# ShigemichiMatsuzaki/MSPL

Measured on AMD Instinct MI355X. Metric: images/sec pseudo-label gen, ESPDNet-UE s=2.0 480x360(->288x480) bs=16, higher is better.
Workload: dtype f32; 1 GPU; BASELINE configs[1]: ESPDNet-UE s=2.0 C=13 single-source pseudo-label gen (forward + pred+0.5aux argmax + KL uncertainty + histogram), bs=16/GPU, 16x3x288x480 fp32, hipGraph replay, 3 launches in flight per GPU, 2 consecutive batches of 16 per launch; per_gpu_batch=16, batches_in_flight=3, batches_per_launch=2, classes=13

## Files before the change

mspl_amd/csrc/pyrpool_stream.hip:

```cpp
#include <stdlib.h>

#include <algorithm>

#include "common.hpp"
#include "pyr_stencil.hpp"

namespace mspl {

constexpr int P3_MAXB = 5;
#ifndef P3_STEPS
#define P3_STEPS 2
#endif
constexpr int P3_SEGMAX = 19;

struct Pyr3Geom {
    int N, P, h, w;
    int hs[P3_MAXB], ws[P3_MAXB];
    float sh[P3_MAXB], sw[P3_MAXB];
    int SEG, nseg, ncb, CBW;
    unsigned total;
};

template <int T, int PXL>
__device__ __forceinline__ void p3_up_branch(const float (&xw)[5][PXL + 4], const float* __restrict__ Arow,
                                             const float (&C)[3][PXL][5], float (&b)[PXL]) {
    constexpr int R0 = (5 - T) / 2;
    constexpr int NCOL = PXL + T - 1;
#pragma unroll
    for (int ky = 0; ky < 3; ++ky) {
        float a[5];
        {
            const float4 t4 = *reinterpret_cast<const float4*>(Arow + ky * 8);
            a[0] = t4.x; a[1] = t4.y; a[2] = t4.z; a[3] = t4.w;
            a[4] = T > 4 ? Arow[ky * 8 + 4] : 0.f;
        }
        float cs[NCOL];
#pragma unroll
        for (int s = 0; s < NCOL; ++s) {
            float v = a[0] * xw[R0][R0 + s];
#pragma unroll
            for (int rr = 1; rr < T; ++rr) v = fmaf(a[rr], xw[R0 + rr][R0 + s], v);
            cs[s] = v;
        }
#pragma unroll
        for (int j = 0; j < PXL; ++j) {
            float v = b[j];
#pragma unroll
            for (int s = 0; s < T; ++s) v = fmaf(C[ky][j][s], cs[j + s], v);
            b[j] = v;
        }
    }
}

template <int PXL> struct P3Vec;
template <> struct P3Vec<1> { typedef float T; };
template <> struct P3Vec<2> { typedef float2 T; };

template <int T0, int T1, int PXL, bool TRAIN>
__global__ __launch_bounds__(256, 2) void pyrpool_stream_kernel(const float* __restrict__ x, const float* __restrict__ sw0,
                                                                const float* __restrict__ sw1, const float* __restrict__ sw2,
                                                                const float* __restrict__ de3, const float* __restrict__ de4,
                                                                const float* __restrict__ br_scale, const float* __restrict__ br_shift,
                                                                const float* __restrict__ br_alpha, const float* __restrict__ merge_w,
                                                                const float* __restrict__ ep_scale,
                                                                const float* __restrict__ ep_shift,
                                                                const float* __restrict__ ep_alpha, int ep_ctot, int ep_coff,
                                                                Pyr3Geom g, float* __restrict__ out, float* __restrict__ zcat,
                                                                float* __restrict__ mraw) {
    __shared__ __attribute__((aligned(16))) float At[2][(P3_SEGMAX + 2) * 24];
    __shared__ float Gt[2][3][PXL][5][64];
    __shared__ __attribute__((aligned(16))) float Wm[4][5][12];
    const int lane = threadIdx.x & 63, wave = __builtin_amdgcn_readfirstlane(threadIdx.x >> 6);
    unsigned bid = blockIdx.x;
    const int sgi = bid % g.nseg;  bid /= g.nseg;
    const int cb = bid % g.ncb;  bid /= g.ncb;
    const int plane = (int)bid * 4 + wave;
    const int n = plane / g.P, c = plane - n * g.P;
    const int h = g.h, w = g.w;
    const int ys = sgi * g.SEG, ye = min(ys + g.SEG, h);
    const int px0 = cb * g.CBW + (lane - 1) * PXL;
    const bool writer = lane >= 1 && lane <= 62 && px0 < w;

    if (wave < 2) {
        const int ri = lane / 3, ky = lane - 3 * ri;
        if (ri < g.SEG + 2) {
            float acc[5];
            if (wave == 0) p3_coeffs<T0>(ys - 1 + ri, ky, h, g.hs[0], g.sh[0], acc);
            else p3_coeffs<T1>(ys - 1 + ri, ky, h, g.hs[1], g.sh[1], acc);
            float* d = &At[wave][ri * 24 + ky * 8];
            d[0] = acc[0]; d[1] = acc[1]; d[2] = acc[2]; d[3] = acc[3]; d[4] = acc[4];
        }
    }
#pragma unroll
    for (int t = 0; t < 6 * PXL; ++t) {
        if ((t & 3) == wave) {
            const int ub = t / (3 * PXL), r = t - ub * 3 * PXL, kx = r / PXL, j = r - kx * PXL;
            float acc[5];
            if (ub == 0) p3_coeffs<T0>(px0 + j, kx, w, g.ws[0], g.sw[0], acc);
            else p3_coeffs<T1>(px0 + j, kx, w, g.ws[1], g.sw[1], acc);
#pragma unroll
            for (int q = 0; q < 5; ++q) Gt[ub][kx][j][q][lane] = acc[q];
        }
    }
    __syncthreads();
    float C0[3][PXL][5], C1[3][PXL][5];
    {
        const float* w0p = sw0 + (size_t)c * 9;
        const float* w1p = sw1 + (size_t)c * 9;
#pragma unroll
        for (int j = 0; j < PXL; ++j)
#pragma unroll
            for (int s2 = 0; s2 < 5; ++s2) {
                const float a0 = Gt[0][0][j][s2][lane], a1 = Gt[0][1][j][s2][lane], a2 = Gt[0][2][j][s2][lane];
                const float b0 = Gt[1][0][j][s2][lane], b1 = Gt[1][1][j][s2][lane], b2 = Gt[1][2][j][s2][lane];
#pragma unroll
                for (int ky = 0; ky < 3; ++ky) {
                    C0[ky][j][s2] = fmaf(w0p[ky * 3 + 2], a2, fmaf(w0p[ky * 3 + 1], a1, w0p[ky * 3] * a0));
                    C1[ky][j][s2] = fmaf(w1p[ky * 3 + 2], b2, fmaf(w1p[ky * 3 + 1], b1, w1p[ky * 3] * b0));
                }
            }
    }
    unsigned dxa[2][PXL], dxb[2][PXL];  float dw0[2][PXL], dw1[2][PXL];
#pragma unroll
    for (int i = 0; i < 2; ++i)
#pragma unroll
        for (int j = 0; j < PXL; ++j) {
            const int px = min(max(px0 + j, 0), w - 1);
            int xa, xb;
            bilinear_src(g.sw[3 + i], px, g.ws[3 + i], xa, xb, dw0[i][j], dw1[i][j]);
            dxa[i][j] = (unsigned)xa * 4u;  dxb[i][j] = (unsigned)xb * 4u;
        }
    const float* wsame = sw2 + (size_t)c * 9;
    if (lane < 45) Wm[wave][lane / 9][lane % 9] = merge_w[(size_t)c * 45 + lane];
    const float4* wmq = reinterpret_cast<const float4*>(&Wm[wave][0][0]);
    float bsc[5], bsh[5], bal[5];
#pragma unroll
    for (int i = 0; i < 5; ++i) { bsc[i] = br_scale[i * g.P + c]; bsh[i] = br_shift[i * g.P + c]; bal[i] = br_alpha[i * g.P + c]; }
    const int cabs = ep_coff + c;
    const float esc = ep_scale ? ep_scale[cabs] : 1.f, esh = ep_shift ? ep_shift[cabs] : 0.f, eal = ep_alpha ? ep_alpha[cabs] : 1.f;
    const unsigned plane_id = __builtin_amdgcn_readfirstlane((unsigned)(n * g.P + c));
    const float* xpl = x + (size_t)plane_id * (size_t)(h * w);
    const float* e3 = de3 + (size_t)plane_id * (size_t)(g.hs[3] * g.ws[3]);
    const float* e4 = de4 + (size_t)plane_id * (size_t)(g.hs[4] * g.ws[4]);
    float* opl = out + ((size_t)__builtin_amdgcn_readfirstlane((unsigned)(n * ep_ctot + cabs))) * (size_t)(h * w);
    bool colin[PXL];
#pragma unroll
    for (int j = 0; j < PXL; ++j) colin[j] = px0 + j >= 0 && px0 + j < w;

    constexpr unsigned P3_OOB = 0x7ffffff0u;
    unsigned xoff[PXL + 4];
#pragma unroll
    for (int j = 0; j < PXL + 4; ++j) {
        const int cx = px0 - 2 + j;
        xoff[j] = (cx >= 0 && cx < w) ? (unsigned)cx * 4u : P3_OOB;
    }
    auto load_row = [&](int r, float (&v)[PXL + 4]) {
        const bool rin = r >= 0 && r < h;
        const float* row = xpl + (size_t)(rin ? r : 0) * w;
        const __amdgpu_buffer_rsrc_t rs = __builtin_amdgcn_make_buffer_rsrc(const_cast<float*>(row), 0, rin ? w * 4 : 0, 0x00020000);
        if (PXL == 2) {
#pragma unroll
            for (int j = 0; j < PXL + 4; j += 2) {
                typedef unsigned u32x2 __attribute__((ext_vector_type(2)));
                const u32x2 t = __builtin_amdgcn_raw_buffer_load_b64(rs, xoff[j], 0, 0);
                v[j] = __uint_as_float(t.x);  v[j + 1] = __uint_as_float(t.y);
            }
        } else {
#pragma unroll
            for (int j = 0; j < PXL + 4; ++j) v[j] = __uint_as_float(__builtin_amdgcn_raw_buffer_load_b32(rs, xoff[j], 0, 0));
        }
    };

    float xw[5][PXL + 4];
#pragma unroll
    for (int rr = 0; rr < 5; ++rr) load_row(ys - 3 + rr, xw[rr]);
    float en[2][PXL][4];
    float enwy0[2], enwy1[2];
    auto load_e = [&](int r) {
#pragma unroll
        for (int i = 0; i < 2; ++i) {
            int ya, yb;
            bilinear_src(g.sh[3 + i], min(max(r, 0), h - 1), g.hs[3 + i], ya, yb, enwy0[i], enwy1[i]);
            const int rowb = g.ws[3 + i] * 4;
            const __amdgpu_buffer_rsrc_t ra = __builtin_amdgcn_make_buffer_rsrc(const_cast<float*>((i == 0 ? e3 : e4) + ya * g.ws[3 + i]), 0, rowb, 0x00020000);
            const __amdgpu_buffer_rsrc_t rb = __builtin_amdgcn_make_buffer_rsrc(const_cast<float*>((i == 0 ? e3 : e4) + yb * g.ws[3 + i]), 0, rowb, 0x00020000);
#pragma unroll
            for (int j = 0; j < PXL; ++j) {
                en[i][j][0] = __uint_as_float(__builtin_amdgcn_raw_buffer_load_b32(ra, dxa[i][j], 0, 0));
                en[i][j][1] = __uint_as_float(__builtin_amdgcn_raw_buffer_load_b32(ra, dxb[i][j], 0, 0));
                en[i][j][2] = __uint_as_float(__builtin_amdgcn_raw_buffer_load_b32(rb, dxa[i][j], 0, 0));
                en[i][j][3] = __uint_as_float(__builtin_amdgcn_raw_buffer_load_b32(rb, dxb[i][j], 0, 0));
            }
        }
    };
    load_e(ys - 1);
    float acc[3][PXL];
#pragma unroll
    for (int r = 0; r < 3; ++r)
#pragma unroll
        for (int j = 0; j < PXL; ++j) acc[r][j] = 0.f;

    auto row_step = [&](const int br) __attribute__((always_inline)) {
        float bv[5][PXL];
        const bool rowin = br >= 0 && br < h;
        float ecur[2][PXL][4], wy0c[2], wy1c[2];
#pragma unroll
        for (int i = 0; i < 2; ++i) {
            wy0c[i] = enwy0[i]; wy1c[i] = enwy1[i];
#pragma unroll
            for (int j = 0; j < PXL; ++j)
#pragma unroll
                for (int q = 0; q < 4; ++q) ecur[i][j][q] = en[i][j][q];
        }
        if (br < ye) load_e(br + 1);
        float xn[PXL + 4];
        load_row(br + 3, xn);
        __builtin_amdgcn_sched_barrier(0);
        if (rowin) {
            const float* A0 = &At[0][(br - (ys - 1)) * 24];
            const float* A1 = &At[1][(br - (ys - 1)) * 24];
#pragma unroll
            for (int j = 0; j < PXL; ++j) { bv[0][j] = 0.f; bv[1][j] = 0.f; bv[2][j] = 0.f; }
            p3_up_branch<T0, PXL>(xw, A0, C0, bv[0]);
            p3_up_branch<T1, PXL>(xw, A1, C1, bv[1]);
#pragma unroll
            for (int ky = 0; ky < 3; ++ky) {
                const float w0 = wsame[ky * 3], w1 = wsame[ky * 3 + 1], w2 = wsame[ky * 3 + 2];
#pragma unroll
                for (int j = 0; j < PXL; ++j) {
                    bv[2][j] = fmaf(w0, xw[1 + ky][j + 1], bv[2][j]);
                    bv[2][j] = fmaf(w1, xw[1 + ky][j + 2], bv[2][j]);
                    bv[2][j] = fmaf(w2, xw[1 + ky][j + 3], bv[2][j]);
                }
            }
#pragma unroll
            for (int i = 0; i < 2; ++i)
#pragma unroll
                for (int j = 0; j < PXL; ++j) {
                    const float top = dw0[i][j] * ecur[i][j][0] + dw1[i][j] * ecur[i][j][1];
                    const float bot = dw0[i][j] * ecur[i][j][2] + dw1[i][j] * ecur[i][j][3];
                    bv[3 + i][j] = wy0c[i] * top + wy1c[i] * bot;
                }
            if (TRAIN && writer && br >= ys && br < ye) {
#pragma unroll
                for (int i = 0; i < 5; ++i) {
                    float* zp = zcat + (((size_t)n * 5 + i) * g.P + c) * (size_t)h * w + (size_t)br * w + px0;
                    if (PXL == 2) *reinterpret_cast<float2*>(zp) = make_float2(bv[i][0], bv[i][PXL - 1]);
                    else zp[0] = bv[i][0];
                }
            }
#pragma unroll
            for (int i = 0; i < 5; ++i)
#pragma unroll
                for (int j = 0; j < PXL; ++j) {
                    float v = fmaf(bv[i][j], bsc[i], bsh[i]);
                    v = v > 0.f ? v : bal[i] * v;
                    bv[i][j] = colin[j] ? v : 0.f;
                }
        } else {
#pragma unroll
            for (int i = 0; i < 5; ++i)
#pragma unroll
                for (int j = 0; j < PXL; ++j) bv[i][j] = 0.f;
        }
#pragma unroll
        for (int i = 0; i < 5; ++i) {
            float bx[PXL + 2];
            bx[0] = p3_from_left(bv[i][PXL - 1]);
#pragma unroll
            for (int j = 0; j < PXL; ++j) bx[1 + j] = bv[i][j];
            bx[PXL + 1] = p3_from_right(bv[i][0]);
            const float4 q0 = wmq[i * 3], q1 = wmq[i * 3 + 1], q2 = wmq[i * 3 + 2];
            const float wv[12] = {q0.x, q0.y, q0.z, q0.w, q1.x, q1.y, q1.z, q1.w, q2.x, q2.y, q2.z, q2.w};
#pragma unroll
            for (int r = 0; r < 3; ++r) {
                const int ky = 2 - r;
                const float w0 = wv[ky * 3], w1 = wv[ky * 3 + 1], w2 = wv[ky * 3 + 2];
#pragma unroll
                for (int j = 0; j < PXL; ++j) {
                    acc[r][j] = fmaf(w0, bx[j], acc[r][j]);
                    acc[r][j] = fmaf(w1, bx[j + 1], acc[r][j]);
                    acc[r][j] = fmaf(w2, bx[j + 2], acc[r][j]);
                }
            }
        }
#pragma unroll
        for (int rr = 0; rr < 4; ++rr)
#pragma unroll
            for (int j = 0; j < PXL + 4; ++j) xw[rr][j] = xw[rr + 1][j];
#pragma unroll
        for (int j = 0; j < PXL + 4; ++j) xw[4][j] = xn[j];
        const int y = br - 1;
        if (y >= ys) {
            float v[PXL];
#pragma unroll
            for (int j = 0; j < PXL; ++j) {
                v[j] = fmaf(acc[0][j], esc, esh);
                v[j] = (ep_alpha && v[j] <= 0.f) ? eal * v[j] : v[j];
            }
            if (writer) {
                float* dst = opl + (size_t)y * w + px0;
                if (PXL == 2) store_out2(dst, make_float2(v[0], v[PXL - 1]));
                else dst[0] = v[0];
                if (TRAIN) {
                    float* rp = mraw + ((size_t)n * g.P + c) * (size_t)h * w + (size_t)y * w + px0;
                    if (PXL == 2) *reinterpret_cast<float2*>(rp) = make_float2(acc[0][0], acc[0][PXL - 1]);
                    else rp[0] = acc[0][0];
                }
            }
        }
#pragma unroll
        for (int j = 0; j < PXL; ++j) { acc[0][j] = acc[1][j]; acc[1][j] = acc[2][j]; acc[2][j] = 0.f; }
    };
    constexpr int STEPS = TRAIN ? 2 : P3_STEPS;
#pragma unroll 1
    for (int br = ys - 1; br <= ye; br += STEPS) {
        row_step(br);
#pragma unroll
        for (int u = 1; u < STEPS; ++u)
            if (br + u <= ye) row_step(br + u);
    }
}

int pyrpool_stream_try(const float* x, int N, int P, int h, int w, int nb, const int32_t* hs, const int32_t* ws,
                       const float* const* stage_w, const float* const* down_e, const float* br_scale,
                       const float* br_shift, const float* br_alpha, const float* merge_w, const Epi& e, float* out,
                       hipStream_t stream, float* zcat) {
    static const int off = (MSPL_TUNE_INT("MSPL_PYR_STREAM", 1) == 0);
    static const int min_w = MSPL_TUNE_INT("MSPL_PYR_STREAM_MINW", 40);
    if (off || nb != 5 || w < min_w || ((int64_t)N * P) % 4 != 0) return 1;
    if (e.pre_add || e.residual || e.reinf_r || e.gate) return 1;
    for (int i = 0; i < 5; ++i) if (hs[i] <= 0 || ws[i] <= 0) return 1;
    if (!(hs[0] > h && ws[0] > w && hs[1] > h && ws[1] > w)) return 1;
    if (!(hs[2] == h && ws[2] == w)) return 1;
    if (!(hs[3] <= h && ws[3] <= w && hs[4] <= h && ws[4] <= w && (hs[3] < h || ws[3] < w) && (hs[4] < h || ws[4] < w))) return 1;
    if (!stage_w[0] || !stage_w[1] || !stage_w[2] || !down_e[3] || !down_e[4]) return 1;
    int taps[2];
    for (int i = 0; i < 2; ++i) {
        const int R = std::max(p3_stencil_radius(h, hs[i]), p3_stencil_radius(w, ws[i]));
        if (R > 2) return 1;
        taps[i] = R <= 1 ? 3 : 5;
    }
    const int PXL = w <= 62 ? 1 : 2;
    if (PXL == 2 && ((w & 1) || (((uintptr_t)out) & 7) || (((uintptr_t)x) & 7))) return 1;
    if (zcat && (!e.raw || e.ctot != P || e.coff != 0)) return 1;
    if (zcat && PXL == 2 && ((((uintptr_t)zcat) | ((uintptr_t)e.raw)) & 7)) return 1;
    Pyr3Geom g;
    memset(&g, 0, sizeof(g));
    g.N = N; g.P = P; g.h = h; g.w = w;
    for (int i = 0; i < 5; ++i) {
        g.hs[i] = hs[i]; g.ws[i] = ws[i];
        if (i < 2) { g.sh[i] = bilinear_scale(h, hs[i]); g.sw[i] = bilinear_scale(w, ws[i]); }
        if (i > 2) { g.sh[i] = bilinear_scale(hs[i], h); g.sw[i] = bilinear_scale(ws[i], w); }
    }
    g.CBW = 62 * PXL;
    g.ncb = ceil_div(w, g.CBW);
    static const int dbg_seg = MSPL_TUNE_INT("MSPL_PYR_SEG", 0);
    int seg = std::min(h, P3_SEGMAX);
    while (seg > 6 && (int64_t)N * P * g.ncb * ceil_div(h, seg) < 2048) --seg;
    seg = ceil_div(h, ceil_div(h, seg));
    if (dbg_seg > 0 && dbg_seg <= P3_SEGMAX) seg = std::min(dbg_seg, h);
    g.SEG = seg;
    g.nseg = ceil_div(h, seg);
    const int64_t waves = (int64_t)N * P * g.ncb * g.nseg;
    if (waves >= (1ll << 31)) return 1;
    g.total = (unsigned)waves;
    const dim3 grid((unsigned)(waves / 4)), blk(256);
#define MSPL_P3_LAUNCH(A, B, L) do { \
        if (zcat) hipLaunchKernelGGL((pyrpool_stream_kernel<A, B, L, true>), grid, blk, 0, stream, x, stage_w[0], stage_w[1], stage_w[2], down_e[3], down_e[4], br_scale, br_shift, br_alpha, merge_w, e.scale, e.shift, e.alpha, e.ctot, e.coff, g, out, zcat, e.raw); \
        else hipLaunchKernelGGL((pyrpool_stream_kernel<A, B, L, false>), grid, blk, 0, stream, x, stage_w[0], stage_w[1], stage_w[2], down_e[3], down_e[4], br_scale, br_shift, br_alpha, merge_w, e.scale, e.shift, e.alpha, e.ctot, e.coff, g, out, (float*)nullptr, (float*)nullptr); } while (0)
    if (PXL == 1) {
        if (taps[0] == 3 && taps[1] == 3) MSPL_P3_LAUNCH(3, 3, 1);
        else if (taps[0] == 3) MSPL_P3_LAUNCH(3, 5, 1);
        else if (taps[1] == 3) MSPL_P3_LAUNCH(5, 3, 1);
        else MSPL_P3_LAUNCH(5, 5, 1);
    } else {
        if (taps[0] == 3 && taps[1] == 3) MSPL_P3_LAUNCH(3, 3, 2);
        else if (taps[0] == 3) MSPL_P3_LAUNCH(3, 5, 2);
        else if (taps[1] == 3) MSPL_P3_LAUNCH(5, 3, 2);
        else MSPL_P3_LAUNCH(5, 5, 2);
    }
#undef MSPL_P3_LAUNCH
    MSPL_CHECK_LAUNCH("pyrpool_fused(streaming form)");
    return MSPL_OK;
}

}
```

Baseline: 21830 images/s.

## Stream pyramid-pool row stencils via scatter accumulators and enlarge row segments

The fused pyramid-pooling kernel stops gathering each output row from a 5-row register window. Each incoming input row is now horizontally filtered once and scattered into per-branch pending accumulators that slide down by one row per step. The shared vertical-coefficient table is re-indexed to per-input-row form, and its fill is spread over all four waves. The default segment height rises from 19 to 36 rows, which cuts halo reloads and per-block setup but adds LDS, prologue work and fewer blocks.

```diff
diff --git a/mspl_amd/csrc/pyrpool_stream.hip b/mspl_amd/csrc/pyrpool_stream.hip
--- a/mspl_amd/csrc/pyrpool_stream.hip
+++ b/mspl_amd/csrc/pyrpool_stream.hip
@@ -11,7 +11,10 @@
 #ifndef P3_STEPS
 #define P3_STEPS 2
 #endif
-constexpr int P3_SEGMAX = 19;
+#ifndef P3_SEGMAX
+#define P3_SEGMAX 36
+#endif
+constexpr int P3_TROWS = P3_SEGMAX + 6;
 
 struct Pyr3Geom {
     int N, P, h, w;
@@ -22,34 +25,56 @@
 };
 
 template <int T, int PXL>
-__device__ __forceinline__ void p3_up_branch(const float (&xw)[5][PXL + 4], const float* __restrict__ Arow,
-                                             const float (&C)[3][PXL][5], float (&b)[PXL]) {
+__device__ __forceinline__ void p3_up_enter(const float (&xr)[PXL + 4], const float* __restrict__ Asrc,
+                                            const float (&C)[3][PXL][5], float (&pend)[T][PXL], const int kmin) {
     constexpr int R0 = (5 - T) / 2;
-    constexpr int NCOL = PXL + T - 1;
 #pragma unroll
     for (int ky = 0; ky < 3; ++ky) {
         float a[5];
         {
-            const float4 t4 = *reinterpret_cast<const float4*>(Arow + ky * 8);
+            const float4 t4 = *reinterpret_cast<const float4*>(Asrc + ky * 8);
             a[0] = t4.x; a[1] = t4.y; a[2] = t4.z; a[3] = t4.w;
-            a[4] = T > 4 ? Arow[ky * 8 + 4] : 0.f;
-        }
-        float cs[NCOL];
-#pragma unroll
-        for (int s = 0; s < NCOL; ++s) {
-            float v = a[0] * xw[R0][R0 + s];
-#pragma unroll
-            for (int rr = 1; rr < T; ++rr) v = fmaf(a[rr], xw[R0 + rr][R0 + s], v);
-            cs[s] = v;
-        }
+            a[4] = T > 4 ? Asrc[ky * 8 + 4] : 0.f;
+        }
+        float hx[PXL];
 #pragma unroll
         for (int j = 0; j < PXL; ++j) {
-            float v = b[j];
-#pragma unroll
-            for (int s = 0; s < T; ++s) v = fmaf(C[ky][j][s], cs[j + s], v);
-            b[j] = v;
-        }
-    }
+            float v = C[ky][j][0] * xr[R0 + j];
+#pragma unroll
+            for (int s = 1; s < T; ++s) v = fmaf(C[ky][j][s], xr[R0 + j + s], v);
+            hx[j] = v;
+        }
+#pragma unroll
+        for (int k = 0; k < T; ++k)
+            if (k >= kmin) {
+#pragma unroll
+                for (int j = 0; j < PXL; ++j) pend[k][j] = (k == T - 1 && ky == 0) ? a[k] * hx[j] : fmaf(a[k], hx[j], pend[k][j]);
+            }
+    }
+}
+
+template <int PXL>
+__device__ __forceinline__ void p3_same_enter(const float (&xr)[PXL + 4], const float* __restrict__ wsame, float (&pend)[3][PXL],
+                                              const int kmin) {
+#pragma unroll
+    for (int k = 0; k < 3; ++k)
+        if (k >= kmin) {
+            const float w0 = wsame[(2 - k) * 3], w1 = wsame[(2 - k) * 3 + 1], w2 = wsame[(2 - k) * 3 + 2];
+#pragma unroll
+            for (int j = 0; j < PXL; ++j) {
+                float v = k == 2 ? w0 * xr[j + 1] : fmaf(w0, xr[j + 1], pend[k][j]);
+                v = fmaf(w1, xr[j + 2], v);
+                pend[k][j] = fmaf(w2, xr[j + 3], v);
+            }
+        }
+}
+
+template <int T, int PXL>
+__device__ __forceinline__ void p3_slide(float (&pend)[T][PXL]) {
+#pragma unroll
+    for (int k = 0; k + 1 < T; ++k)
+#pragma unroll
+        for (int j = 0; j < PXL; ++j) pend[k][j] = pend[k + 1][j];
 }
 
 template <int PXL> struct P3Vec;
@@ -67,7 +92,7 @@
                                                                 const float* __restrict__ ep_alpha, int ep_ctot, int ep_coff,
                                                                 Pyr3Geom g, float* __restrict__ out, float* __restrict__ zcat,
                                                                 float* __restrict__ mraw) {
-    __shared__ __attribute__((aligned(16))) float At[2][(P3_SEGMAX + 2) * 24];
+    __shared__ __attribute__((aligned(16))) float At[2][P3_TROWS * 24];
     __shared__ float Gt[2][3][PXL][5][64];
     __shared__ __attribute__((aligned(16))) float Wm[4][5][12];
     const int lane = threadIdx.x & 63, wave = __builtin_amdgcn_readfirstlane(threadIdx.x >> 6);
@@ -81,15 +106,21 @@
     const int px0 = cb * g.CBW + (lane - 1) * PXL;
     const bool writer = lane >= 1 && lane <= 62 && px0 < w;
 
-    if (wave < 2) {
-        const int ri = lane / 3, ky = lane - 3 * ri;
-        if (ri < g.SEG + 2) {
-            float acc[5];
-            if (wave == 0) p3_coeffs<T0>(ys - 1 + ri, ky, h, g.hs[0], g.sh[0], acc);
-            else p3_coeffs<T1>(ys - 1 + ri, ky, h, g.hs[1], g.sh[1], acc);
-            float* d = &At[wave][ri * 24 + ky * 8];
-            d[0] = acc[0]; d[1] = acc[1]; d[2] = acc[2]; d[3] = acc[3]; d[4] = acc[4];
-        }
+    {
+        const int ub = wave & 1, e = lane / 3, ky = lane - 3 * e;
+        const int R = ((ub == 0 ? T0 : T1) - 1) / 2;
+        if (e < 21)
+            for (int i = (wave >> 1) * 21 + e; i < g.SEG + 2 + 4 * R; i += 42) {
+                const int t = ys - 1 - 2 * R + i;
+                float acc[5];
+                if (ub == 0) p3_coeffs<T0>(t, ky, h, g.hs[0], g.sh[0], acc);
+                else p3_coeffs<T1>(t, ky, h, g.hs[1], g.sh[1], acc);
+#pragma unroll
+                for (int q = 0; q < 5; ++q) {
+                    const int r = t - R + q;
+                    if (q <= 2 * R && r >= ys - 1 - R && r <= ye + R) At[ub][(r - (ys - 3)) * 24 + ky * 8 + 2 * R - q] = acc[q];
+                }
+            }
     }
 #pragma unroll
     for (int t = 0; t < 6 * PXL; ++t) {
@@ -171,9 +202,31 @@
         }
     };
 
-    float xw[5][PXL + 4];
-#pragma unroll
-    for (int rr = 0; rr < 5; ++rr) load_row(ys - 3 + rr, xw[rr]);
+    float pend0[T0][PXL] = {}, pend1[T1][PXL] = {}, pend2[3][PXL] = {};
+    float xw[2][PXL + 4];
+    {
+        float xp[5][PXL + 4];
+#pragma unroll
+        for (int rr = 0; rr < 5; ++rr) load_row(ys - 3 + rr, xp[rr]);
+        constexpr int Ra = (T0 - 1) / 2, Rb = (T1 - 1) / 2;
+#pragma unroll
+        for (int p = 0; p < 2 * Ra; ++p) {
+            p3_up_enter<T0, PXL>(xp[2 - Ra + p], &At[0][(2 - Ra + p) * 24], C0, pend0, 2 * Ra - p);
+            p3_slide<T0, PXL>(pend0);
+        }
+#pragma unroll
+        for (int p = 0; p < 2 * Rb; ++p) {
+            p3_up_enter<T1, PXL>(xp[2 - Rb + p], &At[1][(2 - Rb + p) * 24], C1, pend1, 2 * Rb - p);
+            p3_slide<T1, PXL>(pend1);
+        }
+#pragma unroll
+        for (int p = 0; p < 2; ++p) {
+            p3_same_enter<PXL>(xp[1 + p], wsame, pend2, 2 - p);
+            p3_slide<3, PXL>(pend2);
+        }
+#pragma unroll
+        for (int j = 0; j < PXL + 4; ++j) { xw[0][j] = xp[3][j]; xw[1][j] = xp[4][j]; }
+    }
     float en[2][PXL][4];
     float enwy0[2], enwy1[2];
     auto load_e = [&](int r) {
@@ -201,75 +254,23 @@
         for (int j = 0; j < PXL; ++j) acc[r][j] = 0.f;
 
     auto row_step = [&](const int br) __attribute__((always_inline)) {
-        float bv[5][PXL];
         const bool rowin = br >= 0 && br < h;
-        float ecur[2][PXL][4], wy0c[2], wy1c[2];
-#pragma unroll
-        for (int i = 0; i < 2; ++i) {
-            wy0c[i] = enwy0[i]; wy1c[i] = enwy1[i];
-#pragma unroll
-            for (int j = 0; j < PXL; ++j)
-#pragma unroll
-                for (int q = 0; q < 4; ++q) ecur[i][j][q] = en[i][j][q];
-        }
-        if (br < ye) load_e(br + 1);
-        float xn[PXL + 4];
-        load_row(br + 3, xn);
-        __builtin_amdgcn_sched_barrier(0);
-        if (rowin) {
-            const float* A0 = &At[0][(br - (ys - 1)) * 24];
-            const float* A1 = &At[1][(br - (ys - 1)) * 24];
-#pragma unroll
-            for (int j = 0; j < PXL; ++j) { bv[0][j] = 0.f; bv[1][j] = 0.f; bv[2][j] = 0.f; }
-            p3_up_branch<T0, PXL>(xw, A0, C0, bv[0]);
-            p3_up_branch<T1, PXL>(xw, A1, C1, bv[1]);
-#pragma unroll
-            for (int ky = 0; ky < 3; ++ky) {
-                const float w0 = wsame[ky * 3], w1 = wsame[ky * 3 + 1], w2 = wsame[ky * 3 + 2];
-#pragma unroll
-                for (int j = 0; j < PXL; ++j) {
-                    bv[2][j] = fmaf(w0, xw[1 + ky][j + 1], bv[2][j]);
-                    bv[2][j] = fmaf(w1, xw[1 + ky][j + 2], bv[2][j]);
-                    bv[2][j] = fmaf(w2, xw[1 + ky][j + 3], bv[2][j]);
-                }
-            }
-#pragma unroll
-            for (int i = 0; i < 2; ++i)
-#pragma unroll
-                for (int j = 0; j < PXL; ++j) {
-                    const float top = dw0[i][j] * ecur[i][j][0] + dw1[i][j] * ecur[i][j][1];
-                    const float bot = dw0[i][j] * ecur[i][j][2] + dw1[i][j] * ecur[i][j][3];
-                    bv[3 + i][j] = wy0c[i] * top + wy1c[i] * bot;
-                }
+        auto merge_in = [&](const int i, const float (&z)[PXL]) __attribute__((always_inline)) {
+            if (!rowin) return;
             if (TRAIN && writer && br >= ys && br < ye) {
-#pragma unroll
-                for (int i = 0; i < 5; ++i) {
-                    float* zp = zcat + (((size_t)n * 5 + i) * g.P + c) * (size_t)h * w + (size_t)br * w + px0;
-                    if (PXL == 2) *reinterpret_cast<float2*>(zp) = make_float2(bv[i][0], bv[i][PXL - 1]);
-                    else zp[0] = bv[i][0];
-                }
-            }
-#pragma unroll
-            for (int i = 0; i < 5; ++i)
-#pragma unroll
-                for (int j = 0; j < PXL; ++j) {
-                    float v = fmaf(bv[i][j], bsc[i], bsh[i]);
-                    v = v > 0.f ? v : bal[i] * v;
-                    bv[i][j] = colin[j] ? v : 0.f;
-                }
-        } else {
-#pragma unroll
-            for (int i = 0; i < 5; ++i)
-#pragma unroll
-                for (int j = 0; j < PXL; ++j) bv[i][j] = 0.f;
-        }
-#pragma unroll
-        for (int i = 0; i < 5; ++i) {
+                float* zp = zcat + (((size_t)n * 5 + i) * g.P + c) * (size_t)h * w + (size_t)br * w + px0;
+                if (PXL == 2) *reinterpret_cast<float2*>(zp) = make_float2(z[0], z[PXL - 1]);
+                else zp[0] = z[0];
+            }
             float bx[PXL + 2];
-            bx[0] = p3_from_left(bv[i][PXL - 1]);
-#pragma unroll
-            for (int j = 0; j < PXL; ++j) bx[1 + j] = bv[i][j];
-            bx[PXL + 1] = p3_from_right(bv[i][0]);
+#pragma unroll
+            for (int j = 0; j < PXL; ++j) {
+                float v = fmaf(z[j], bsc[i], bsh[i]);
+                v = v > 0.f ? v : bal[i] * v;
+                bx[1 + j] = colin[j] ? v : 0.f;
+            }
+            bx[0] = p3_from_left(bx[PXL]);
+            bx[PXL + 1] = p3_from_right(bx[1]);
             const float4 q0 = wmq[i * 3], q1 = wmq[i * 3 + 1], q2 = wmq[i * 3 + 2];
             const float wv[12] = {q0.x, q0.y, q0.z, q0.w, q1.x, q1.y, q1.z, q1.w, q2.x, q2.y, q2.z, q2.w};
 #pragma unroll
@@ -283,13 +284,36 @@
                     acc[r][j] = fmaf(w2, bx[j + 2], acc[r][j]);
                 }
             }
-        }
-#pragma unroll
-        for (int rr = 0; rr < 4; ++rr)
-#pragma unroll
-            for (int j = 0; j < PXL + 4; ++j) xw[rr][j] = xw[rr + 1][j];
-#pragma unroll
-        for (int j = 0; j < PXL + 4; ++j) xw[4][j] = xn[j];
+        };
+        float dn[2][PXL];
+#pragma unroll
+        for (int i = 0; i < 2; ++i)
+#pragma unroll
+            for (int j = 0; j < PXL; ++j) {
+                const float top = dw0[i][j] * en[i][j][0] + dw1[i][j] * en[i][j][1];
+                const float bot = dw0[i][j] * en[i][j][2] + dw1[i][j] * en[i][j][3];
+                dn[i][j] = enwy0[i] * top + enwy1[i] * bot;
+            }
+        if (br < ye) load_e(br + 1);
+        float xn[PXL + 4];
+        load_row(br + 3, xn);
+        __builtin_amdgcn_sched_barrier(0);
+        p3_up_enter<T0, PXL>(xw[(T0 - 1) / 2 - 1], &At[0][(br + (T0 - 1) / 2 - (ys - 3)) * 24], C0, pend0, 0);
+        merge_in(0, pend0[0]);
+        __builtin_amdgcn_sched_barrier(0);
+        p3_up_enter<T1, PXL>(xw[(T1 - 1) / 2 - 1], &At[1][(br + (T1 - 1) / 2 - (ys - 3)) * 24], C1, pend1, 0);
+        merge_in(1, pend1[0]);
+        __builtin_amdgcn_sched_barrier(0);
+        p3_same_enter<PXL>(xw[0], wsame, pend2, 0);
+        merge_in(2, pend2[0]);
+        __builtin_amdgcn_sched_barrier(0);
+        merge_in(3, dn[0]);
+        merge_in(4, dn[1]);
+        p3_slide<T0, PXL>(pend0);
+        p3_slide<T1, PXL>(pend1);
+        p3_slide<3, PXL>(pend2);
+#pragma unroll
+        for (int j = 0; j < PXL + 4; ++j) { xw[0][j] = xw[1][j]; xw[1][j] = xn[j]; }
         const int y = br - 1;
         if (y >= ys) {
             float v[PXL];
```

Result: no change. 22000 images/s (median of 6 runs) (+0.8%).
